# vliu15/3d-brain-tumor-segmentation

Hardware: AMD Instinct MI355X
Metric: training volumes/sec (2ch x 128^3) (higher is better)
Workload: dtype f32; 1 GPU; BASELINE configs[1]: 2ch x 128^3, batch 1 per GPU, fp32, full fwd+bwd with Dice+KL+L2 VAE loss + Dice metric + TF-form Adam; CLI-default model (base_filters=32, depth=4, groups=8, reduction=8; 42,174,773 params); parallelism=dp1, global_batch=1

## Files before the change

3d-brain-tumor-segmentation_amd/csrc/conv_igemm.hip:

```cpp
#include <stdlib.h>
#include "common.h"
#include "conv_plan.h"

#define MAXSLOT 8

int bts_prof_on();
void bts_prof_begin(int sym, double flops, hipStream_t stream);
void bts_prof_end(hipStream_t stream);

struct IgemmParams {
  const float* x;
  const float* wp;
  const float* bias;
  float* y;
  int N, Di, Hi, Wi, Cin, ldx;
  int Do, Ho, Wo;
  int Cout, ldy, Npad, KG;
  int ODa, OHa, OWa;
  int os, ooz, ooy, oox;
  int s, loz, loy, lox;
  int IZ, IY, IX;
  int lgTX, lgTY, TZ;
  int ntz, nty, ntx;
  int ntaps, flags;
// ... 811 lines not shown
#pragma unroll
    for (int i = 0; i < UPM_NSLOT; ++i) {
      f32x4 v = {0.f, 0.f, 0.f, 0.f};
      if (goff[i] >= 0) v = *reinterpret_cast<const f32x4*>(xbase + goff[i] + st * 8);
      pre[i] = v;
    }
  };
  auto commit = [&](float* buf) {
#pragma unroll
    for (int i = 0; i < UPM_NSLOT; ++i) {
      const int e = tid + i * 256;
      if (e < nslots) *reinterpret_cast<f32x4*>(buf + (e >> 1) * S + (e & 1) * 4) = pre[i];
    }
  };
  int kgBeg = 0, kgEnd = p.KG;
  if (p.ksplit > 1) {
    kgBeg = blockIdx.z * p.kg_per;
    kgEnd = kgBeg + p.kg_per;
    if (kgEnd > p.KG) kgEnd = p.KG;
  }
  fetch(kgBeg);
  commit(lds);
  __syncthreads();
  for (int st = kgBeg; st < kgEnd; ++st) {
    const float* cur = lds + ((st - kgBeg) & 1) * bufDw;
    const bool more = (st + 1) < kgEnd;
    if (more) fetch(st + 1);
    const float* wk = p.wp + st * wstepKG;
    constexpr int AD = 2;
    f32x4 a[AD + 1], bf[8];
#pragma unroll
    for (int q = 0; q < AD; ++q) a[q] = *reinterpret_cast<const f32x4*>((wk + q * wstepTap) + lane_woff);
#pragma unroll
    for (int o = 0; o < 8; ++o) bf[o] = *reinterpret_cast<const f32x4*>(cur + bbase + off8[o]);
#pragma unroll
    for (int t = 0; t < 27; ++t) {
      if (t + AD < 27) a[(t + AD) % (AD + 1)] = *reinterpret_cast<const f32x4*>((wk + (t + AD) * wstepTap) + lane_woff);
      __builtin_amdgcn_sched_barrier(0);
#pragma unroll
      for (int j = 0; j < 4; ++j)
        acc[upm_cls(t)] = __builtin_amdgcn_mfma_f32_32x32x2f32(a[t % (AD + 1)][j], bf[upm_off(t)][j], acc[upm_cls(t)], 0, 0, 0);
      __builtin_amdgcn_sched_barrier(0);
    }
    if (more) commit(lds + ((st + 1 - kgBeg) & 1) * bufDw);
    __syncthreads();
  }

  const int cz = cz0 + mz, cy = cy0 + my, cx = cx0 + mx;
  if (cz >= p.Di || cy >= p.Hi || cx >= p.Wi) return;
  const int nb = blockIdx.y * 32;
#pragma unroll
  for (int c = 0; c < 8; ++c) {
    const int oz = 2 * cz + ((c >> 2) & 1), oy = 2 * cy + ((c >> 1) & 1), ox = 2 * cx + (c & 1);
    const long vfine = (((long)n * (2 * p.Di) + oz) * (2 * p.Hi) + oy) * (2 * p.Wi) + ox;
    if (p.ksplit > 1) {
      float* row = p.part + ((long)blockIdx.z * ((long)p.N * 8 * p.Di * p.Hi * p.Wi) + vfine) * p.Npad;
#pragma unroll
      for (int g = 0; g < 4; ++g) {
        f32x4 v4 = {acc[c][4 * g + 0], acc[c][4 * g + 1], acc[c][4 * g + 2], acc[c][4 * g + 3]};
        *reinterpret_cast<f32x4*>(row + nb + 8 * g + 4 * h) = v4;
      }
      continue;
    }
    float* yrow = p.y + vfine * (long)p.ldy;
#pragma unroll
    for (int g = 0; g < 4; ++g) {
      const int co = nb + 8 * g + 4 * h;
      if (co >= p.Cout) continue;
      f32x4 v = {acc[c][4 * g + 0], acc[c][4 * g + 1], acc[c][4 * g + 2], acc[c][4 * g + 3]};
      if (p.flags & IG_FLAG_BIAS) {
#pragma unroll
        for (int j = 0; j < 4; ++j) v[j] += p.bias[co + j];
      }
      if (p.flags & IG_FLAG_SIGMOID) {
#pragma unroll
        for (int j = 0; j < 4; ++j) v[j] = sigmoidf_(v[j]);
      }
      f32x4* dst = reinterpret_cast<f32x4*>(yrow + co);
      if (p.flags & IG_FLAG_ACCUM) v += *dst;
      *dst = v;
    }
  }
}

static bool upm_accept(const ConvCall& c, ConvChoice& ch) {
  UpmPlan& u = ch.u;
  if ((c.ldx & 3) || (c.ldy & 3) || !c.x16 || !c.y16) return false;
  if ((c.Cin & 7) || (c.Cout & 3) || c.Wi < 8 || c.Hi < 4 || c.Di < 2) return false;
  const int Npad = npad32(c.Cout), KG = c.Cin / 8;
  int TX = 32;
  while (TX > 8 && TX / 2 >= c.Wi) TX /= 2;
  int TY = (TX == 32) ? 2 : 4;
  int TZ = 128 / (TX * TY);
  u.lgTX = ilog2(TX); u.lgTY = ilog2(TY); u.TZ = TZ;
  u.ntx = (c.Wi + TX - 1) / TX; u.nty = (c.Hi + TY - 1) / TY; u.ntz = (c.Di + TZ - 1) / TZ;
  u.IX = TX + 1; u.IY = TY + 1; u.IZ = TZ + 1;
  if (u.IZ * u.IY * u.IX * 2 > 256 * UPM_NSLOT) return false;
  const long wgs = (long)c.N * u.ntz * u.nty * u.ntx * (Npad / 32);
  const long min_wgs = conv_env_long("BTS_IGEMM_UPM_MIN", 256);
  u.ksplit = 1; u.kg_per = KG; u.need = 0;
  if (wgs < min_wgs) {
    if (KG < 8) return false;
    int ks = (int)((512 + wgs - 1) / wgs);
    if (ks > KG / 4) ks = KG / 4;
    if (ks > 16) ks = 16;
    if (ks < 2) return false;
    u.kg_per = (KG + ks - 1) / ks;
    u.ksplit = (KG + u.kg_per - 1) / u.kg_per;
    if (u.ksplit < 2 || wgs * u.ksplit < min_wgs / 2) return false;
    u.need = (long)u.ksplit * c.N * 8 * c.Di * c.Hi * c.Wi * Npad * 4;
  }
  ch.sym = 20;
  ch.ws = u.need;
  return c.ws_bytes >= u.need;
}

static int launch_upm(const ConvCall& c, const ConvChoice& ch, const ConvPtrs& q, hipStream_t stream) {
  const UpmPlan& u = ch.u;
  UpmParams p;
  p.N = c.N; p.Di = c.Di; p.Hi = c.Hi; p.Wi = c.Wi; p.Cin = c.Cin; p.Cout = c.Cout;
  p.Npad = npad32(c.Cout); p.KG = c.Cin / 8;
  p.lgTX = u.lgTX; p.lgTY = u.lgTY; p.TZ = u.TZ; p.ntx = u.ntx; p.nty = u.nty; p.ntz = u.ntz; p.IX = u.IX; p.IY = u.IY; p.IZ = u.IZ;
  p.ksplit = u.ksplit; p.kg_per = u.kg_per;
  p.x = q.x; p.wp = q.wp; p.bias = q.bias; p.y = q.y; p.ldx = c.ldx; p.ldy = c.ldy; p.flags = c.flags;
  p.part = reinterpret_cast<float*>(q.ws);
  const long tiles = (long)c.N * p.ntz * p.nty * p.ntx;
  const int ny = p.Npad / 32;
  const int tileVox = p.IZ * p.IY * p.IX;
  const size_t shmem = (size_t)2 * tileVox * 12 * sizeof(float);
  const bool prof = bts_prof_on();
  if (prof) bts_prof_begin(20, 2.0 * 27.0 * c.Cin * c.Cout * (double)c.N * c.Di * c.Hi * c.Wi, stream);
  (void)hipGetLastError(); hipLaunchKernelGGL(upm_kernel, dim3((unsigned)tiles, ny, p.ksplit), dim3(256), shmem, stream, p);
  if (prof) bts_prof_end(stream);
  BTS_LAUNCH_CHECK();
  if (p.ksplit > 1) {
    const long nvox = (long)c.N * 8 * c.Di * c.Hi * c.Wi;
    long blocks = (nvox * c.Cout + 255) / 256;
    if (blocks > 4096) blocks = 4096;
    (void)hipGetLastError(); hipLaunchKernelGGL(igemm_reduce_kernel, dim3((int)blocks), dim3(256), 0, stream, p.part, q.bias, q.y, nvox, c.Cout, p.Npad,
                       c.ldy, p.ksplit, p.flags);
    BTS_LAUNCH_CHECK();
  }
  return BTS_OK;
}

struct K1sParams {
  const float* x;
  const float* wp;
  const float* bias;
  float* y;
  long nvox;
  int Cin, ldx, Cout, ldy, Npad, KG, flags;
};
template <int NS>
__global__ __launch_bounds__(256, 4) void k1s_kernel(const K1sParams p) {
  const int lane = threadIdx.x & 63;
  const int wave = __builtin_amdgcn_readfirstlane(threadIdx.x >> 6);
  const int h = lane >> 5, l32 = lane & 31;
  const long v0 = (long)blockIdx.x * 256 + wave * 64;
  const float* xrow[2];
#pragma unroll
  for (int ms = 0; ms < 2; ++ms) {
    long v = v0 + ms * 32 + l32;
    if (v >= p.nvox) v = p.nvox - 1;
    xrow[ms] = p.x + v * p.ldx + h * 4;
  }
  int woff[NS];
#pragma unroll
  for (int ns = 0; ns < NS; ++ns) {
    int ncol = (blockIdx.y * NS + ns) * 32 + l32;
    if (ncol >= p.Npad) ncol = p.Npad - 1;
    woff[ns] = (h * p.Npad + ncol) * 4;
  }
  const int wstepKG = 2 * p.Npad * 4;
  f32x16 acc[2][NS];
#pragma unroll
  for (int ms = 0; ms < 2; ++ms)
#pragma unroll
    for (int ns = 0; ns < NS; ++ns)
#pragma unroll
      for (int r = 0; r < 16; ++r) acc[ms][ns][r] = 0.f;
  constexpr int U = (NS == 1) ? 2 : 1;
  f32x4 b[2][U][2], a[2][U][NS];
  auto load = [&](int buf, int kg) {
#pragma unroll
    for (int u = 0; u < U; ++u) {
      const int k = (kg + u < p.KG) ? kg + u : p.KG - 1;
#pragma unroll
      for (int ms = 0; ms < 2; ++ms) b[buf][u][ms] = *reinterpret_cast<const f32x4*>(xrow[ms] + k * 8);
#pragma unroll
      for (int ns = 0; ns < NS; ++ns) a[buf][u][ns] = *reinterpret_cast<const f32x4*>((p.wp + k * wstepKG) + woff[ns]);
    }
  };
  auto mma = [&](int buf, int kg) {
#pragma unroll
    for (int u = 0; u < U; ++u) {
      if (kg + u < p.KG) {
#pragma unroll
        for (int j = 0; j < 4; ++j)
#pragma unroll
          for (int ms = 0; ms < 2; ++ms)
#pragma unroll
            for (int ns = 0; ns < NS; ++ns)
              acc[ms][ns] = __builtin_amdgcn_mfma_f32_32x32x2f32(a[buf][u][ns][j], b[buf][u][ms][j], acc[ms][ns], 0, 0, 0);
      }
    }
  };
  load(0, 0);
  for (int kg = 0; kg < p.KG; kg += 2 * U) {
    if (kg + U < p.KG) load(1, kg + U);
    mma(0, kg);
    if (kg + U < p.KG) {
      if (kg + 2 * U < p.KG) load(0, kg + 2 * U);
      mma(1, kg + U);
    }
  }
#pragma unroll
  for (int ms = 0; ms < 2; ++ms) {
    const long v = v0 + ms * 32 + l32;
    if (v >= p.nvox) continue;
    float* yrow = p.y + v * p.ldy;
#pragma unroll
    for (int ns = 0; ns < NS; ++ns) {
      const int nb = (blockIdx.y * NS + ns) * 32;
#pragma unroll
      for (int g = 0; g < 4; ++g) {
        const int co = nb + 8 * g + 4 * h;
        if (co >= p.Cout) continue;
        f32x4 val = {acc[ms][ns][4 * g + 0], acc[ms][ns][4 * g + 1], acc[ms][ns][4 * g + 2], acc[ms][ns][4 * g + 3]};
        if (p.flags & IG_FLAG_BIAS) {
#pragma unroll
          for (int j = 0; j < 4; ++j)
            if (co + j < p.Cout) val[j] += p.bias[co + j];
        }
        if (p.flags & IG_FLAG_SIGMOID) {
#pragma unroll
          for (int j = 0; j < 4; ++j) val[j] = sigmoidf_(val[j]);
        }
        if ((p.flags & IG_FLAG_VECOUT) && co + 3 < p.Cout) {
          f32x4* dst = reinterpret_cast<f32x4*>(yrow + co);
          if (p.flags & IG_FLAG_ACCUM) val += *dst;
          *dst = val;
        } else {
#pragma unroll
          for (int j = 0; j < 4; ++j)
            if (co + j < p.Cout) yrow[co + j] = (p.flags & IG_FLAG_ACCUM) ? yrow[co + j] + val[j] : val[j];
        }
      }
    }
  }
}

static bool k1s_accept(const ConvCall& c, ConvChoice& ch) {
  if ((c.Cin & 7) || (c.ldx & 3) || !c.x16) return false;
  const long nvox = (long)c.N * c.Di * c.Hi * c.Wi;
  if (nvox < conv_env_long("BTS_IGEMM_K1S_MIN", 256 * 256)) return false;
  ch.sym = 21;
  return (nvox + 255) / 256 <= 0x7fffffffL;
}
static int launch_k1s(const ConvCall& c, const ConvChoice&, const ConvPtrs& q, hipStream_t stream) {
  K1sParams p;
  p.x = q.x; p.wp = q.wp; p.bias = q.bias; p.y = q.y; p.nvox = (long)c.N * c.Di * c.Hi * c.Wi;
  p.Cin = c.Cin; p.ldx = c.ldx; p.Cout = c.Cout; p.ldy = c.ldy; p.Npad = npad32(c.Cout); p.KG = c.Cin / 8;
  p.flags = c.flags;
  if ((c.ldy % 4 == 0) && c.y16) p.flags |= IG_FLAG_VECOUT;
  const long gx = (p.nvox + 255) / 256;
  const bool prof = bts_prof_on();
  const int ns = (p.Npad >= 64) ? 2 : 1;
  if (prof) bts_prof_begin(21, 2.0 * c.Cin * (double)c.Cout * (double)p.nvox, stream);
  (void)hipGetLastError();
  if (ns == 2) hipLaunchKernelGGL(k1s_kernel<2>, dim3((unsigned)gx, (p.Npad + 63) / 64), dim3(256), 0, stream, p);
  else hipLaunchKernelGGL(k1s_kernel<1>, dim3((unsigned)gx, 1), dim3(256), 0, stream, p);
  if (prof) bts_prof_end(stream);
  BTS_LAUNCH_CHECK();
  return BTS_OK;
}

struct DscParams {
  const float* x;
  const float* wp;
  const float* bias;
  float* y;
  int N, D, H, W, Cin, ldx, Cout, ldy, Npad, KG, ntx, nty, ntz, flags;
};
template <int CO>
__global__ __launch_bounds__(256, 4) void dsc_kernel(const DscParams p) {
  constexpr int S = 12, TX = 32, TY = 4, TZ = 2, IX = TX + 2, IY = TY + 2, IZ = TZ + 2;
  constexpr int tileVox = IZ * IY * IX, nslots = tileVox * 2, NSL = (nslots + 255) / 256;
  __shared__ __attribute__((aligned(16))) float lds[tileVox * S];
  const int tid = threadIdx.x;
  int b = blockIdx.x;
  const int tx = b % p.ntx; b /= p.ntx;
  const int ty = b % p.nty; b /= p.nty;
  const int tz = b % p.ntz;
  const int n = b / p.ntz;
  const int iz0 = tz * TZ - 1, iy0 = ty * TY - 1, ix0 = tx * TX - 1;
  const float* xbase = p.x + ((((long)n * p.D + iz0) * p.H + iy0) * p.W + ix0) * (long)p.ldx;
  int goff[NSL];
#pragma unroll
  for (int i = 0; i < NSL; ++i) {
    const int e = tid + i * 256;
    goff[i] = -1;
    if (e < nslots) {
      const int vox = e >> 1, q = e & 1;
      const int vz = vox / (IY * IX), r = vox - vz * (IY * IX), vy = r / IX, vx = r - vy * IX;
      if ((unsigned)(iz0 + vz) < (unsigned)p.D && (unsigned)(iy0 + vy) < (unsigned)p.H && (unsigned)(ix0 + vx) < (unsigned)p.W)
        goff[i] = ((vz * p.H + vy) * p.W + vx) * p.ldx + q * 4;
    }
  }
  const int mx = tid & (TX - 1), my = (tid >> 5) & (TY - 1), mz = tid >> 7;
  const float* lb = lds + ((mz * IY + my) * IX + mx) * S;
  float acc[CO];
#pragma unroll
  for (int c = 0; c < CO; ++c) acc[c] = 0.f;
  const int wstepKG = 2 * p.Npad * 4, wstepTap = p.KG * wstepKG;
  f32x4 pre[NSL];
  auto fetch = [&](int kg) {
#pragma unroll
    for (int i = 0; i < NSL; ++i) {
      f32x4 v = {0.f, 0.f, 0.f, 0.f};
      if (goff[i] >= 0) v = *reinterpret_cast<const f32x4*>(xbase + goff[i] + kg * 8);
      pre[i] = v;
    }
  };
  fetch(0);
  for (int kg = 0; kg < p.KG; ++kg) {
    __syncthreads();
#pragma unroll
    for (int i = 0; i < NSL; ++i) {
      const int e = tid + i * 256;
      if (e < nslots) *reinterpret_cast<f32x4*>(lds + (e >> 1) * S + (e & 1) * 4) = pre[i];
    }
    __syncthreads();
    if (kg + 1 < p.KG) fetch(kg + 1);
    const float* wk = p.wp + kg * wstepKG;
#pragma unroll
    for (int r = 0; r < 9; ++r) {
      float w[3][2][CO * 4];
#pragma unroll
      for (int dx = 0; dx < 3; ++dx)
#pragma unroll
        for (int hh = 0; hh < 2; ++hh)
#pragma unroll
          for (int q = 0; q < CO * 4; ++q) w[dx][hh][q] = wk[(r * 3 + dx) * wstepTap + hh * p.Npad * 4 + q];
      f32x4 xv[3][2];
#pragma unroll
      for (int dx = 0; dx < 3; ++dx) {
        const float* src = lb + (((r / 3) * IY + r % 3) * IX + dx) * S;
        xv[dx][0] = *reinterpret_cast<const f32x4*>(src);
        xv[dx][1] = *reinterpret_cast<const f32x4*>(src + 4);
      }
      __builtin_amdgcn_sched_barrier(0);
#pragma unroll
      for (int dx = 0; dx < 3; ++dx)
#pragma unroll
        for (int hh = 0; hh < 2; ++hh)
#pragma unroll
          for (int c = 0; c < CO; ++c)
#pragma unroll
            for (int j = 0; j < 4; ++j) acc[c] = fmaf(xv[dx][hh][j], w[dx][hh][c * 4 + j], acc[c]);
      __builtin_amdgcn_sched_barrier(0);
    }
  }
  const int oz = tz * TZ + mz, oy = ty * TY + my, ox = tx * TX + mx;
  if (oz >= p.D || oy >= p.H || ox >= p.W) return;
  float* yrow = p.y + ((((long)n * p.D + oz) * p.H + oy) * p.W + ox) * (long)p.ldy;
#pragma unroll
  for (int c = 0; c < CO; ++c) {
    if (c < p.Cout) {
      float v = acc[c];
      if (p.flags & IG_FLAG_BIAS) v += p.bias[c];
      if (p.flags & IG_FLAG_SIGMOID) v = sigmoidf_(v);
      if (p.flags & IG_FLAG_ACCUM) v += yrow[c];
      yrow[c] = v;
    }
  }
}

static bool dsc_accept(const ConvCall& c, ConvChoice& ch) {
  if (c.Cout > 4 || (c.Cin & 7) || (c.ldx & 3) || !c.x16) return false;
  const long tiles = (long)c.N * ((c.Di + 1) / 2) * ((c.Hi + 3) / 4) * ((c.Wi + 31) / 32);
  ch.sym = 22;
  return tiles >= conv_env_long("BTS_IGEMM_DSC_MIN", 1024) && tiles <= 0x7fffffffL;
}
static int launch_dsc(const ConvCall& c, const ConvChoice&, const ConvPtrs& q, hipStream_t stream) {
  DscParams p;
  p.x = q.x; p.wp = q.wp; p.bias = q.bias; p.y = q.y;
  p.N = c.N; p.D = c.Di; p.H = c.Hi; p.W = c.Wi; p.Cin = c.Cin; p.ldx = c.ldx; p.Cout = c.Cout; p.ldy = c.ldy;
  p.Npad = npad32(c.Cout); p.KG = c.Cin / 8;
  p.ntx = (c.Wi + 31) / 32; p.nty = (c.Hi + 3) / 4; p.ntz = (c.Di + 1) / 2;
  p.flags = c.flags;
  const long tiles = (long)c.N * p.ntz * p.nty * p.ntx;
  const bool prof = bts_prof_on();
  if (prof) bts_prof_begin(22, 2.0 * 27.0 * c.Cin * (double)c.Cout * (double)c.N * c.Di * c.Hi * c.Wi, stream);
  (void)hipGetLastError();
  if (c.Cout <= 2) hipLaunchKernelGGL(dsc_kernel<2>, dim3((unsigned)tiles), dim3(256), 0, stream, p);
  else hipLaunchKernelGGL(dsc_kernel<4>, dim3((unsigned)tiles), dim3(256), 0, stream, p);
  if (prof) bts_prof_end(stream);
  BTS_LAUNCH_CHECK();
  return BTS_OK;
}

struct C2Params {
  const float* x;
  const float* wp;
  const float* bias;
  float* y;
  const float* wp2;
  const float* bias2;
  float* y2;
  int N, D, H, W, ldx, Cout, ldy, ldy2, Npad;
  int ntz, nty, ntx;
  double* gnp;
  int gn_G, gn_zt;
};

template <bool F2>
__global__ __launch_bounds__(256, 2) void c2_kernel(const C2Params p) {
  __shared__ float lds[2 * 6 * 6 * 34 + 16];
  const int tid = threadIdx.x;
  const int lane = tid & 63;
  const int wave = __builtin_amdgcn_readfirstlane(tid >> 6);
  const int h = lane >> 5, l32 = lane & 31;
  int b = blockIdx.x;
  const int tx = b % p.ntx; b /= p.ntx;
// ... 592 lines not shown
```

3d-brain-tumor-segmentation_amd/csrc/conv_wgrad.hip:

```cpp
#include <stdlib.h>
#include <type_traits>
#include "common.h"
#include "bts_internal.h"

int bts_prof_on();
void bts_prof_begin(int sym, double flops, hipStream_t stream);
void bts_prof_end(hipStream_t stream);

#define WG_THREADS 512
#define WG_WAVES 8
#define WG_MAXT 4
#define WG_PSLOTS 8
#define WG_QSLOTS 4

struct WgradParams {
  const float* p;
  const float* q;
  float* partial;
  double* partial_b;
  const float* zeros;
  int N, Dp, Hp, Wp, Cp, ldp;
  int Dq, Hq, Wq, Cq, ldq;
  int s, loz, loy, lox;
  int IZ, IY, IX;
// ... 869 lines not shown
    for (int c = 0; c < 4; ++c)
#pragma unroll
      for (int r = 0; r < 16; ++r) acc[a][c][r] = 0.f;

  struct WgwOps {
    f32x4 v[4];
    f32x4 a0, a1, u1, u2;
    float a0s[2], a1s[2], u1s[2], u2s[2];
  };
  auto form = [&](const float* cur, auto stc, WgwOps& o) {
    constexpr int st = decltype(stc)::value;
    constexpr int py2 = st >> 1, sx = st & 1;
    const int xq = 2 * sx + hh;
    const int xo = 4 * xq;
    const int pq = (xq ^ pswz) << 2;
    f32x4 c[4];
#pragma unroll
    for (int yr = 0; yr < 4; ++yr) {
      const f32x4 a = *reinterpret_cast<const f32x4*>(cur + pA + (2 * py2 + yr) * 512 + pq);
      const f32x4 b = *reinterpret_cast<const f32x4*>(cur + pB + (2 * py2 + yr) * 512 + pq);
      c[yr] = wgw_fma4(b, sp2, a);
    }
    o.v[0] = wgw_sub4(c[0], c[2]);
    o.v[1] = wgw_add4(c[1], c[2]);
    o.v[2] = wgw_sub4(c[2], c[1]);
    o.v[3] = wgw_sub4(c[1], c[3]);
    const float* qb = cur + WGW_PTILE + ((2 * py2) * 32 + ch) * WGW_QSTR + xo;
    {
      const f32x4 x0q = *reinterpret_cast<const f32x4*>(qb + qX + 4);
      const f32x4 x1q = *reinterpret_cast<const f32x4*>(qb + qX + 32 * WGW_QSTR + 4);
      const f32x4 y0q = *reinterpret_cast<const f32x4*>(qb + (4 * 32) * WGW_QSTR + 4);
      const f32x4 y1q = *reinterpret_cast<const f32x4*>(qb + (5 * 32) * WGW_QSTR + 4);
      o.a0 = wgw_fma4(y0q, sq2, x0q);
      o.a1 = wgw_fma4(y1q, sq2, x1q);
      o.u1 = wgw_add4(o.a0, o.a1);
      o.u2 = wgw_sub4(o.a0, o.a1);
      if (bias) bsum += (double)((o.u1[0] + o.u1[1]) + (o.u1[2] + o.u1[3]));
    }
#pragma unroll
    for (int e = 0; e < 2; ++e) {
      const int off = e == 0 ? 0 : 8, el = e == 0 ? 3 : 0;
      f32x4 xs0 = *reinterpret_cast<const f32x4*>(qb + qX + off);
      f32x4 xs1 = *reinterpret_cast<const f32x4*>(qb + qX + 32 * WGW_QSTR + off);
      f32x4 ys0 = *reinterpret_cast<const f32x4*>(qb + (4 * 32) * WGW_QSTR + off);
      f32x4 ys1 = *reinterpret_cast<const f32x4*>(qb + (5 * 32) * WGW_QSTR + off);
      asm volatile("" : "+v"(xs0), "+v"(xs1), "+v"(ys0), "+v"(ys1));
      o.a0s[e] = fmaf(ys0[el], sq, xs0[el]);
      o.a1s[e] = fmaf(ys1[el], sq, xs1[el]);
      o.u1s[e] = o.a0s[e] + o.a1s[e];
      o.u2s[e] = o.a0s[e] - o.a1s[e];
    }
  };
  auto mfma48 = [&](const WgwOps& o) {
#pragma unroll
    for (int dx = 0; dx < 3; ++dx)
#pragma unroll
      for (int j = 0; j < 4; ++j) {
        const int w = 5 + j - dx;
        const float b0 = w == 3 ? o.a0s[0] : w == 8 ? o.a0s[1] : o.a0[(w - 4) & 3];
        const float b1 = w == 3 ? o.u1s[0] : w == 8 ? o.u1s[1] : o.u1[(w - 4) & 3];
        const float b2 = w == 3 ? o.u2s[0] : w == 8 ? o.u2s[1] : o.u2[(w - 4) & 3];
        const float b3 = w == 3 ? o.a1s[0] : w == 8 ? o.a1s[1] : o.a1[(w - 4) & 3];
        acc[dx][0] = __builtin_amdgcn_mfma_f32_32x32x2f32(o.v[0][j], b0, acc[dx][0], 0, 0, 0);
        acc[dx][1] = __builtin_amdgcn_mfma_f32_32x32x2f32(o.v[1][j], b1, acc[dx][1], 0, 0, 0);
        acc[dx][2] = __builtin_amdgcn_mfma_f32_32x32x2f32(o.v[2][j], b2, acc[dx][2], 0, 0, 0);
        acc[dx][3] = __builtin_amdgcn_mfma_f32_32x32x2f32(o.v[3][j], b3, acc[dx][3], 0, 0, 0);
      }
  };
#define WGW_SCHED_STEP()                                   \
  _Pragma("unroll") for (int q_ = 0; q_ < 48; ++q_) {      \
    __builtin_amdgcn_sched_group_barrier(0x008, 1, 0);     \
    __builtin_amdgcn_sched_group_barrier(0x002, 2, 0);     \
    __builtin_amdgcn_sched_group_barrier(0x320, 1, 0);     \
  }

  const int t0 = blockIdx.x * p.sub_per_wg;
  int t1 = t0 + p.sub_per_wg;
  if (t1 > p.nsub) t1 = p.nsub;
  if (t0 < t1) {
    fetch_begin();
    fetch_quarter(IC<0>{}); fetch_quarter(IC<1>{}); fetch_quarter(IC<2>{}); fetch_quarter(IC<3>{});
    commit_quarter(lds, IC<0>{}); commit_quarter(lds, IC<1>{}); commit_quarter(lds, IC<2>{}); commit_quarter(lds, IC<3>{});
  }
  __syncthreads();
  WgwOps opA, opB;
  for (int t = t0; t < t1; ++t) {
    const float* cur = lds + ((t - t0) & 1) * WGW_BUF;
    float* nxt = lds + ((t - t0 + 1) & 1) * WGW_BUF;
    const bool more = (t + 1) < t1;
    form(cur, IC<0>{}, opA);
    if (more) fetch_begin();
    __builtin_amdgcn_sched_barrier(0);
    asm volatile("s_nop 3" ::: "memory");
    if (more) fetch_quarter(IC<0>{});
    form(cur, IC<1>{}, opB);
    mfma48(opA);
    WGW_SCHED_STEP();
    __builtin_amdgcn_sched_barrier(0);
    asm volatile("s_nop 1" ::: "memory");
    if (more) { commit_quarter(nxt, IC<0>{}); fetch_quarter(IC<1>{}); }
    form(cur, IC<2>{}, opA);
    mfma48(opB);
    WGW_SCHED_STEP();
    __builtin_amdgcn_sched_barrier(0);
    asm volatile("s_nop 1" ::: "memory");
    if (more) { commit_quarter(nxt, IC<1>{}); fetch_quarter(IC<2>{}); }
    form(cur, IC<3>{}, opB);
    mfma48(opA);
    WGW_SCHED_STEP();
    __builtin_amdgcn_sched_barrier(0);
    asm volatile("s_nop 1" ::: "memory");
    if (more) { commit_quarter(nxt, IC<2>{}); fetch_quarter(IC<3>{}); }
    mfma48(opB);
    WGW_SCHED_STEP();
    __builtin_amdgcn_sched_barrier(0);
    if (more) commit_quarter(nxt, IC<3>{});
    __syncthreads();
  }

  asm volatile("s_nop 15\n\ts_nop 15\n\ts_nop 15\n\ts_nop 15\n\ts_nop 15" ::: "memory");
  float* xl = lds + wave * 9 * 1024;
#pragma unroll
  for (int dx = 0; dx < 3; ++dx)
#pragma unroll
    for (int r = 0; r < 16; ++r) {
      const float u0 = wgw_acc_rd(acc[dx][0][r]), u1 = wgw_acc_rd(acc[dx][1][r]), u2 = wgw_acc_rd(acc[dx][2][r]),
                  u3 = wgw_acc_rd(acc[dx][3][r]);
      const float hs = 0.5f * (u1 + u2), hd = 0.5f * (u1 - u2);
      const int crow = 8 * (r >> 2) + 4 * hh + (r & 3);
      float* o = xl + (dx * 3) * 1024 + crow * 32 + ch;
      o[0] = u0 + hs;
      o[1024] = hd;
      o[2048] = hs - u3;
    }
  __syncthreads();
  float* out = p.partial + ((((long)blockIdx.x * gridDim.y + pct) * gridDim.z + qct) * 27) * 1024;
  for (int e = tid; e < 9 * 1024; e += WGW_THREADS) {
    const int g = e >> 10, ck = e & 1023;
    const int dx = g / 3, ky = g - dx * 3;
    const float l0 = lds[(0 * 9 + g) * 1024 + ck], l1 = lds[(1 * 9 + g) * 1024 + ck], l2 = lds[(2 * 9 + g) * 1024 + ck],
                l3 = lds[(3 * 9 + g) * 1024 + ck];
    const float hs = 0.5f * (l1 + l2), hd = 0.5f * (l1 - l2);
    out[((0 * 3 + ky) * 3 + dx) * 1024 + ck] = l0 + hs;
    out[((1 * 3 + ky) * 3 + dx) * 1024 + ck] = hd;
    out[((2 * 3 + ky) * 3 + dx) * 1024 + ck] = hs - l3;
  }
  if (bias) {
    const double o = __shfl_xor(bsum, 32, 64);
    if (lane < 32) p.partial_b[((long)blockIdx.x * gridDim.z + qct) * 32 + ch] = bsum + o;
  }
}

#define K1W_THREADS 512
#define K1W_U 8
__global__ __launch_bounds__(K1W_THREADS, 2) void k1w_kernel(const WgradParams p, long NV, long chunk) {
  __shared__ float lds[8 * 1024];
  const int tid = threadIdx.x;
  const int lane = tid & 63;
  const int wave = __builtin_amdgcn_readfirstlane(tid >> 6);
  const int ch = lane & 31, hh = lane >> 5;
  const int pct = blockIdx.y, qct = blockIdx.z;
  const int pc = pct * 32 + ch, qc = qct * 32 + ch;
  const bool pok = pc < p.Cp, qok = qc < p.Cq;
  const long w0 = (long)blockIdx.x * chunk;
  long w1 = w0 + chunk;
  if (w1 > NV) w1 = NV;
  long per = ((w1 - w0 + 7) / 8 + 1) & ~1L;
  long v = w0 + wave * per;
  long ve = v + per;
  if (ve > w1) ve = w1;
  f32x16 acc;
#pragma unroll
  for (int r = 0; r < 16; ++r) acc[r] = 0.f;
  double bsum = 0.0;
  const bool bias = p.want_bias && pct == 0;
  const float* pp = p.p + pc;
  const float* qq = p.q + qc;
  for (; v < ve; v += 2 * K1W_U) {
    float a[K1W_U], b[K1W_U];
#pragma unroll
    for (int u = 0; u < K1W_U; ++u) {
      const long vv = v + 2 * u + hh;
      const bool in = vv < ve;
      a[u] = (in && pok) ? pp[vv * p.ldp] : 0.f;
      b[u] = (in && qok) ? qq[vv * p.ldq] : 0.f;
    }
    float bs = 0.f;
#pragma unroll
    for (int u = 0; u < K1W_U; ++u) {
      acc = __builtin_amdgcn_mfma_f32_32x32x2f32(a[u], b[u], acc, 0, 0, 0);
      bs += b[u];
    }
    if (bias) bsum += (double)bs;
  }
#pragma unroll
  for (int r = 0; r < 16; ++r) lds[wave * 1024 + ((r & 3) + 8 * (r >> 2) + 4 * hh) * 32 + ch] = acc[r];
  __syncthreads();
  float* dst = p.partial + ((((long)blockIdx.x * gridDim.y + pct) * gridDim.z + qct) * p.ntiles) * 1024;
  for (int e = tid; e < 1024; e += K1W_THREADS) {
    float sacc = lds[e];
#pragma unroll
    for (int w = 1; w < 8; ++w) sacc += lds[w * 1024 + e];
    dst[e] = sacc;
  }
  if (bias) {
    __syncthreads();
    double* shd = reinterpret_cast<double*>(lds);
    shd[tid] = bsum;
    __syncthreads();
    if (tid < 32) {
      double t = 0.0;
      for (int k = 0; k < 16; ++k) t += shd[k * 32 + tid];
      p.partial_b[((long)blockIdx.x * gridDim.z + qct) * 32 + tid] = t;
    }
  }
}

struct WgradRoles {
  int ntaps, s, neg, swapped, transposed;
  int Dp, Hp, Wp, Cp, Dq, Hq, Wq, Cq;
};

static int wgrad_roles(WgradRoles& r, int kind, int D, int H, int W, int Cin, int Cout) {
  r.ntaps = (kind == BTS_CONV_K1) ? 1 : 27;
  r.s = 1; r.neg = 0; r.swapped = 0; r.transposed = 0;
  r.Dp = D; r.Hp = H; r.Wp = W; r.Cp = Cin; r.Dq = D; r.Hq = H; r.Wq = W; r.Cq = Cout;
  if (kind == BTS_CONV_K3S2) {
    if ((D | H | W) & 1) return BTS_ERR_SHAPE;
    r.s = 2; r.Dq = D / 2; r.Hq = H / 2; r.Wq = W / 2;
  } else if (kind == BTS_CONV_K3S2T) {
    r.transposed = 1;
    r.s = 2; r.Dp = 2 * D; r.Hp = 2 * H; r.Wp = 2 * W; r.Cp = Cout; r.Cq = Cin;
  } else if (kind == BTS_CONV_K3S1 && Cout <= 8 && Cin > Cout) {
    r.swapped = 1; r.neg = 1; r.Cp = Cout; r.Cq = Cin;
  }
  return BTS_OK;
}

extern "C" int bts_colsum(const float* x, float* out, void* workspace, long workspace_bytes, int N, long rows, int C,
                          int ld, float scale, int sum_over_n, int accumulate, hipStream_t stream);
extern "C" long bts_colsum_workspace(int N, long rows, int C);

extern "C" long bts_conv3d_bwd_weight_workspace(int kind, int N, int D, int H, int W, int Cin, int Cout) {
  WgradRoles r;
  if (wgrad_roles(r, kind, D, H, W, Cin, Cout) != BTS_OK) return -1;
  WgradPlan pl;
  if (plan_wgrad(pl, r.ntaps, r.s, r.neg, N, r.Dp, r.Hp, r.Wp, r.Cp, r.Dq, r.Hq, r.Wq, r.Cq) != BTS_OK) return -1;
  const long base = ((pl.partial_floats * 4 + pl.partial_b_doubles * 8 + 256 + 15) & ~15L);
  return base + (r.swapped ? bts_colsum_workspace(N, (long)D * H * W, Cout) : 0) + 128;
}

extern "C" int bts_conv3d_bwd_weight(int kind, const float* x, const float* dy, float* dw, float* db, void* workspace,
                                     long workspace_bytes, int N, int D, int H, int W, int Cin, int ldx, int Cout,
                                     int lddy, int dup_start, int dup_shift, int accumulate, hipStream_t stream) {
  WgradRoles ro;
  int r = wgrad_roles(ro, kind, D, H, W, Cin, Cout);
  if (r != BTS_OK) return r;
  if (dup_shift > 0 && (kind == BTS_CONV_K3S2 || kind == BTS_CONV_K3S2T)) return BTS_ERR_UNSUPPORTED;
  WgradPlan pl;
  r = plan_wgrad(pl, ro.ntaps, ro.s, ro.neg, N, ro.Dp, ro.Hp, ro.Wp, ro.Cp, ro.Dq, ro.Hq, ro.Wq, ro.Cq);
  if (r != BTS_OK) return r;
  const long need = bts_conv3d_bwd_weight_workspace(kind, N, D, H, W, Cin, Cout);
  if (workspace_bytes < need || workspace == nullptr) return BTS_ERR_WORKSPACE;
  WgradParams& p = pl.p;
  const bool pIsDy = ro.transposed || ro.swapped;
  p.p = pIsDy ? dy : x;
  p.q = pIsDy ? x : dy;
  p.ldp = pIsDy ? lddy : ldx;
  p.ldq = pIsDy ? ldx : lddy;
  p.partial = reinterpret_cast<float*>(workspace);
  uintptr_t pb = (uintptr_t)(p.partial + pl.partial_floats);
  pb = (pb + 15) & ~(uintptr_t)15;
  p.partial_b = reinterpret_cast<double*>(pb);
  p.want_bias = (db != nullptr && !pIsDy) ? 1 : 0;
  typedef void (*WgKernel)(const WgradParams);
  static const WgKernel kernels[4] = {wgrad_kernel<0, 0>, wgrad_kernel<1, 0>, wgrad_kernel<2, 1>, wgrad_kernel<2, 2>};
  static bool attr_done = false;
  if (!attr_done) {
    for (int i = 0; i < 4; ++i) {
      hipError_t e = hipFuncSetAttribute(reinterpret_cast<const void*>(kernels[i]), hipFuncAttributeMaxDynamicSharedMemorySize, 160 * 1024);
      if (e != hipSuccess) return (int)e;
    }
    attr_done = true;
  }
  char* ztail = reinterpret_cast<char*>(workspace) + ((need - 64) & ~15L);
  p.zeros = reinterpret_cast<const float*>(ztail);
  const bool glds = (p.ldp % 4 == 0) && (p.Cp % 4 == 0) && ((((uintptr_t)p.p) & 15) == 0) && (p.ldq % 4 == 0) &&
                    (p.Cq % 4 == 0) && ((((uintptr_t)p.q) & 15) == 0);
  if (p.fastf && ((double)p.IZ * p.Hp * p.Wp * p.ldp * 4.0 >= 4.0e9 || (double)p.TZ * p.Hq * p.Wq * p.ldq * 4.0 >= 4.0e9 || !glds))
    p.fastf = p.fixg = 0;
  const bool prof = bts_prof_on();
  if (glds && !p.fastf) {
    hipError_t e = hipMemsetAsync(ztail, 0, 64, stream);
    if (e != hipSuccess) return (int)e;
  }
  const int kidx = !glds ? 0 : (p.fastf ? 1 + p.fixg : 1);
  bool use_wgw = false;
  if (kidx == 2 && ro.ntaps == 27 && ro.s == 1) {
    const char* e = getenv("BTS_WGW");
    use_wgw = !(e && atoi(e) == 0) && 5.0 * p.Hp * p.Wp * p.ldp * 4.0 < 2.0e9 && 3.0 * p.Hq * p.Wq * p.ldq * 4.0 < 2.0e9;
  }
  bool use_k1w = false;
  const long NVall = (long)N * ro.Dq * ro.Hq * ro.Wq;
  if (ro.ntaps == 1 && !pIsDy && p.ntiles == 1 && NVall >= 32768) {
    const char* e = getenv("BTS_K1W");
    use_k1w = !(e && atoi(e) == 0);
  }
  if (use_k1w) {
    const long chunk = (((NVall + pl.nsp - 1) / pl.nsp) + 15) & ~15L;
    if (prof) bts_prof_begin(26, 2.0 * (double)ro.Cp * ro.Cq * (double)NVall, stream);
    (void)hipGetLastError();
    hipLaunchKernelGGL(k1w_kernel, dim3(pl.nsp, pl.npct, pl.nqct), dim3(K1W_THREADS), 0, stream, p, NVall, chunk);
    if (prof) bts_prof_end(stream);
    BTS_LAUNCH_CHECK();
  } else if (use_wgw) {
    static bool wattr = false;
    if (!wattr) {
      hipError_t e = hipFuncSetAttribute(reinterpret_cast<const void*>(wgw_kernel), hipFuncAttributeMaxDynamicSharedMemorySize, 160 * 1024);
      if (e != hipSuccess) return (int)e;
      wattr = true;
    }
    if (prof) bts_prof_begin(24, 2.0 * ro.ntaps * (double)ro.Cp * ro.Cq * (double)N * ro.Dq * ro.Hq * ro.Wq, stream);
    (void)hipGetLastError();
    hipLaunchKernelGGL(wgw_kernel, dim3(pl.nsp, pl.npct, pl.nqct), dim3(WGW_THREADS), (size_t)2 * WGW_BUF * sizeof(float), stream, p);
    if (prof) bts_prof_end(stream);
    BTS_LAUNCH_CHECK();
  } else {
  static const int ksym[4] = {100, 104, 109, 110};
  if (prof) bts_prof_begin(ksym[kidx], 2.0 * ro.ntaps * (double)ro.Cp * ro.Cq * (double)N * ro.Dq * ro.Hq * ro.Wq, stream);
  (void)hipGetLastError(); hipLaunchKernelGGL(kernels[kidx], dim3(pl.nsp, pl.npct, pl.nqct), dim3(WG_THREADS), pl.shmem, stream, p);
  if (prof) bts_prof_end(stream);
  BTS_LAUNCH_CHECK();
  }
  WfinParams f;
  f.partial = p.partial; f.partial_b = p.partial_b; f.dw = dw; f.db = p.want_bias ? db : nullptr;
  f.nsp = pl.nsp; f.npct = pl.npct; f.nqct = pl.nqct; f.ntaps = ro.ntaps; f.ntiles = p.ntiles; f.cpad = p.cpad;
  f.Cp = ro.Cp; f.Cq = ro.Cq;
  const int Cin_ref = Cin + dup_shift;
  f.sT = (long)Cin_ref * Cout;
  if (ro.transposed) { f.sP = Cin_ref; f.sQ = 1; f.fold_axis = 0; }
  else if (ro.swapped) { f.sP = 1; f.sQ = Cout; f.fold_axis = 2; }
  else { f.sP = Cout; f.sQ = 1; f.fold_axis = 1; }
  f.shift = dup_shift;
  f.dup_start = dup_shift > 0 ? dup_start : (1 << 30);
  f.accum = accumulate;
  long rows = (long)ro.ntaps * ro.Cp * pl.nqct;
  if (pl.nsp <= 16) {
    long blocks = (rows * 32 + 255) / 256;
    if (blocks > 8192) blocks = 8192;
    (void)hipGetLastError(); hipLaunchKernelGGL(wgrad_finalize_flat_kernel, dim3((int)blocks), dim3(256), 0, stream, f);
  } else {
    int blocks = (int)(rows < 4096 ? rows : 4096);
    (void)hipGetLastError(); hipLaunchKernelGGL(wgrad_finalize_kernel, dim3(blocks), dim3(256), 0, stream, f);
  }
  BTS_LAUNCH_CHECK();
  if (db != nullptr && ro.swapped) {
    char* cw = reinterpret_cast<char*>(workspace) + ((pl.partial_floats * 4 + pl.partial_b_doubles * 8 + 256 + 15) & ~15L);
    const long rowsv = (long)D * H * W;
    return bts_colsum(dy, db, cw, bts_colsum_workspace(N, rowsv, Cout), N, rowsv, Cout, lddy, 1.0f, 1, accumulate, stream);
  }
  return BTS_OK;
}
```

Before: 27.29 volumes/s.

## Restructure 1x1 conv kernels: hold B in registers, pipeline A loads, XCD-aware wgrad mapping

```diff
diff --git a/3d-brain-tumor-segmentation_amd/csrc/conv_igemm.hip b/3d-brain-tumor-segmentation_amd/csrc/conv_igemm.hip
--- a/3d-brain-tumor-segmentation_amd/csrc/conv_igemm.hip
+++ b/3d-brain-tumor-segmentation_amd/csrc/conv_igemm.hip
@@ -987,82 +987,66 @@
   long nvox;
   int Cin, ldx, Cout, ldy, Npad, KG, flags;
 };
-template <int NS>
+template <int NS, int KH>
 __global__ __launch_bounds__(256, 4) void k1s_kernel(const K1sParams p) {
+  constexpr bool HOLD = (NS == 1);
+  constexpr int RA = HOLD ? (KH == 8 ? 2 : 4) : KH;
+  constexpr int OB = HOLD ? (KH == 8 ? 2 : 4) : 2;
   const int lane = threadIdx.x & 63;
   const int wave = __builtin_amdgcn_readfirstlane(threadIdx.x >> 6);
   const int h = lane >> 5, l32 = lane & 31;
   const long v0 = (long)blockIdx.x * 256 + wave * 64;
   const float* xrow[2];
+  float* ycur[2];
+  bool vok[2];
 #pragma unroll
   for (int ms = 0; ms < 2; ++ms) {
     long v = v0 + ms * 32 + l32;
-    if (v >= p.nvox) v = p.nvox - 1;
+    vok[ms] = v < p.nvox;
+    if (!vok[ms]) v = p.nvox - 1;
     xrow[ms] = p.x + v * p.ldx + h * 4;
-  }
-  int woff[NS];
-#pragma unroll
-  for (int ns = 0; ns < NS; ++ns) {
-    int ncol = (blockIdx.y * NS + ns) * 32 + l32;
-    if (ncol >= p.Npad) ncol = p.Npad - 1;
-    woff[ns] = (h * p.Npad + ncol) * 4;
-  }
+    ycur[ms] = p.y + v * p.ldy + h * 4 + blockIdx.y * (32 * NS);
+  }
+  int co0 = blockIdx.y * (32 * NS) + h * 4;
   const int wstepKG = 2 * p.Npad * 4;
-  f32x16 acc[2][NS];
-#pragma unroll
-  for (int ms = 0; ms < 2; ++ms)
-#pragma unroll
-    for (int ns = 0; ns < NS; ++ns)
-#pragma unroll
-      for (int r = 0; r < 16; ++r) acc[ms][ns][r] = 0.f;
-  constexpr int U = (NS == 1) ? 2 : 1;
-  f32x4 b[2][U][2], a[2][U][NS];
-  auto load = [&](int buf, int kg) {
-#pragma unroll
-    for (int u = 0; u < U; ++u) {
-      const int k = (kg + u < p.KG) ? kg + u : p.KG - 1;
-#pragma unroll
-      for (int ms = 0; ms < 2; ++ms) b[buf][u][ms] = *reinterpret_cast<const f32x4*>(xrow[ms] + k * 8);
-#pragma unroll
-      for (int ns = 0; ns < NS; ++ns) a[buf][u][ns] = *reinterpret_cast<const f32x4*>((p.wp + k * wstepKG) + woff[ns]);
-    }
+  const unsigned aoff = (h * p.Npad + l32) * 4;
+  const int lastcb = p.Npad / 32 - 1;
+  f32x4 b[KH][2], a[RA][NS];
+  auto loadB = [&](int slot, int k) {
+#pragma unroll
+    for (int ms = 0; ms < 2; ++ms) b[slot][ms] = *reinterpret_cast<const f32x4*>(xrow[ms] + k * 8);
   };
-  auto mma = [&](int buf, int kg) {
-#pragma unroll
-    for (int u = 0; u < U; ++u) {
-      if (kg + u < p.KG) {
-#pragma unroll
-        for (int j = 0; j < 4; ++j)
-#pragma unroll
-          for (int ms = 0; ms < 2; ++ms)
-#pragma unroll
-            for (int ns = 0; ns < NS; ++ns)
-              acc[ms][ns] = __builtin_amdgcn_mfma_f32_32x32x2f32(a[buf][u][ns][j], b[buf][u][ms][j], acc[ms][ns], 0, 0, 0);
-      }
+  auto loadA = [&](int slot, int cb, int k) {
+#pragma unroll
+    for (int ns = 0; ns < NS; ++ns) {
+      const int c32 = (cb * NS + ns < lastcb) ? cb * NS + ns : lastcb;
+      const float* wk = p.wp + (long)k * wstepKG + c32 * 128;
+      a[slot][ns] = *reinterpret_cast<const f32x4*>(wk + aoff);
     }
   };
-  load(0, 0);
-  for (int kg = 0; kg < p.KG; kg += 2 * U) {
-    if (kg + U < p.KG) load(1, kg + U);
-    mma(0, kg);
-    if (kg + U < p.KG) {
-      if (kg + 2 * U < p.KG) load(0, kg + 2 * U);
-      mma(1, kg + U);
-    }
-  }
-#pragma unroll
-  for (int ms = 0; ms < 2; ++ms) {
-    const long v = v0 + ms * 32 + l32;
-    if (v >= p.nvox) continue;
-    float* yrow = p.y + v * p.ldy;
-#pragma unroll
-    for (int ns = 0; ns < NS; ++ns) {
-      const int nb = (blockIdx.y * NS + ns) * 32;
-#pragma unroll
-      for (int g = 0; g < 4; ++g) {
-        const int co = nb + 8 * g + 4 * h;
-        if (co >= p.Cout) continue;
-        f32x4 val = {acc[ms][ns][4 * g + 0], acc[ms][ns][4 * g + 1], acc[ms][ns][4 * g + 2], acc[ms][ns][4 * g + 3]};
+  const bool vec = (p.flags & IG_FLAG_VECOUT) != 0, accum = (p.flags & IG_FLAG_ACCUM) != 0;
+  const bool rdold = vec && accum && p.Cout >= 4;
+  auto store_tile = [&](const f32x16& c, int ms, int d0) {
+#pragma unroll
+    for (int q0 = 0; q0 < 4; q0 += OB) {
+      __builtin_amdgcn_sched_barrier(0);
+      f32x4 old[OB];
+#pragma unroll
+      for (int i = 0; i < OB; ++i) old[i] = f32x4{0.f, 0.f, 0.f, 0.f};
+      if (rdold) {
+#pragma unroll
+        for (int i = 0; i < OB; ++i) {
+          const int d = d0 + 8 * (q0 + i);
+          old[i] = *reinterpret_cast<const f32x4*>(ycur[ms] + ((co0 + d + 3 < p.Cout) ? d : -co0));
+        }
+      }
+#pragma unroll
+      for (int i = 0; i < OB; ++i) {
+        const int g = q0 + i, d = d0 + 8 * g;
+        const int co = co0 + d;
+        if (!vok[ms] || co >= p.Cout) continue;
+        float* yq = ycur[ms] + d;
+        f32x4 val = {c[4 * g + 0], c[4 * g + 1], c[4 * g + 2], c[4 * g + 3]};
         if (p.flags & IG_FLAG_BIAS) {
 #pragma unroll
           for (int j = 0; j < 4; ++j)
@@ -1072,17 +1056,86 @@
 #pragma unroll
           for (int j = 0; j < 4; ++j) val[j] = sigmoidf_(val[j]);
         }
-        if ((p.flags & IG_FLAG_VECOUT) && co + 3 < p.Cout) {
-          f32x4* dst = reinterpret_cast<f32x4*>(yrow + co);
-          if (p.flags & IG_FLAG_ACCUM) val += *dst;
-          *dst = val;
+        if (vec && co + 3 < p.Cout) {
+          if (accum) val += old[i];
+          *reinterpret_cast<f32x4*>(yq) = val;
         } else {
 #pragma unroll
           for (int j = 0; j < 4; ++j)
-            if (co + j < p.Cout) yrow[co + j] = (p.flags & IG_FLAG_ACCUM) ? yrow[co + j] + val[j] : val[j];
+            if (co + j < p.Cout) yq[j] = accum ? yq[j] + val[j] : val[j];
         }
       }
     }
+  };
+#pragma unroll
+  for (int s = 0; s < RA; ++s) {
+    loadA(s, blockIdx.y, s < p.KG ? s : p.KG - 1);
+    __builtin_amdgcn_sched_barrier(0);
+  }
+#pragma unroll
+  for (int s = 0; s < KH; ++s) {
+    loadB(s, s < p.KG ? s : p.KG - 1);
+    __builtin_amdgcn_sched_barrier(0);
+  }
+  if constexpr (HOLD) {
+    const int nblk = p.Npad / 32;
+    for (int blk = 0; blk < nblk; ++blk) {
+#pragma unroll
+      for (int ms = 0; ms < 2; ++ms) {
+        f32x16 acc;
+#pragma unroll
+        for (int r = 0; r < 16; ++r) acc[r] = 0.f;
+#pragma unroll
+        for (int s = 0; s < KH; ++s) {
+          if (s < p.KG) {
+#pragma unroll
+            for (int j = 0; j < 4; ++j) acc = __builtin_amdgcn_mfma_f32_32x32x2f32(a[s % RA][0][j], b[s][ms][j], acc, 0, 0, 0);
+            if (s + RA < p.KG) loadA(s % RA, blk, s + RA);
+          }
+        }
+        __builtin_amdgcn_sched_barrier(0);
+        if (ms == 0 || blk + 1 < nblk) {
+#pragma unroll
+          for (int s = 0; s < RA; ++s) loadA(s, blk + ms, s < p.KG ? s : p.KG - 1);
+        }
+        store_tile(acc, ms, 0);
+        __builtin_amdgcn_sched_barrier(0);
+      }
+#pragma unroll
+      for (int ms = 0; ms < 2; ++ms) ycur[ms] += 32;
+      co0 += 32;
+    }
+  } else {
+    const int cb = blockIdx.y;
+    f32x16 acc[2][NS];
+#pragma unroll
+    for (int ms = 0; ms < 2; ++ms)
+#pragma unroll
+      for (int ns = 0; ns < NS; ++ns)
+#pragma unroll
+        for (int r = 0; r < 16; ++r) acc[ms][ns][r] = 0.f;
+    for (int kg0 = 0; kg0 < p.KG; kg0 += KH) {
+#pragma unroll
+      for (int s = 0; s < KH; ++s) {
+        const int kg = kg0 + s;
+        if (kg < p.KG) {
+#pragma unroll
+          for (int j = 0; j < 4; ++j)
+#pragma unroll
+            for (int ms = 0; ms < 2; ++ms)
+#pragma unroll
+              for (int ns = 0; ns < NS; ++ns)
+                acc[ms][ns] = __builtin_amdgcn_mfma_f32_32x32x2f32(a[s % RA][ns][j], b[s][ms][j], acc[ms][ns], 0, 0, 0);
+          if (kg + RA < p.KG) loadA(s % RA, cb, kg + RA);
+          if (kg + KH < p.KG) loadB(s, kg + KH);
+        }
+      }
+    }
+    __builtin_amdgcn_sched_barrier(0);
+#pragma unroll
+    for (int ms = 0; ms < 2; ++ms)
+#pragma unroll
+      for (int ns = 0; ns < NS; ++ns) store_tile(acc[ms][ns], ms, ns * 32);
   }
 }
 
@@ -1101,11 +1154,11 @@
   if ((c.ldy % 4 == 0) && c.y16) p.flags |= IG_FLAG_VECOUT;
   const long gx = (p.nvox + 255) / 256;
   const bool prof = bts_prof_on();
-  const int ns = (p.Npad >= 64) ? 2 : 1;
   if (prof) bts_prof_begin(21, 2.0 * c.Cin * (double)c.Cout * (double)p.nvox, stream);
   (void)hipGetLastError();
-  if (ns == 2) hipLaunchKernelGGL(k1s_kernel<2>, dim3((unsigned)gx, (p.Npad + 63) / 64), dim3(256), 0, stream, p);
-  else hipLaunchKernelGGL(k1s_kernel<1>, dim3((unsigned)gx, 1), dim3(256), 0, stream, p);
+  if (p.KG <= 4) hipLaunchKernelGGL((k1s_kernel<1, 4>), dim3((unsigned)gx, 1), dim3(256), 0, stream, p);
+  else if (p.KG <= 8) hipLaunchKernelGGL((k1s_kernel<1, 8>), dim3((unsigned)gx, 1), dim3(256), 0, stream, p);
+  else hipLaunchKernelGGL((k1s_kernel<2, 3>), dim3((unsigned)gx, (p.Npad + 63) / 64), dim3(256), 0, stream, p);
   if (prof) bts_prof_end(stream);
   BTS_LAUNCH_CHECK();
   return BTS_OK;
diff --git a/3d-brain-tumor-segmentation_amd/csrc/conv_wgrad.hip b/3d-brain-tumor-segmentation_amd/csrc/conv_wgrad.hip
--- a/3d-brain-tumor-segmentation_amd/csrc/conv_wgrad.hip
+++ b/3d-brain-tumor-segmentation_amd/csrc/conv_wgrad.hip
@@ -1045,17 +1045,22 @@
 }
 
 #define K1W_THREADS 512
-#define K1W_U 8
-__global__ __launch_bounds__(K1W_THREADS, 2) void k1w_kernel(const WgradParams p, long NV, long chunk) {
+#define K1W_U 32
+__global__ __launch_bounds__(K1W_THREADS, 2) void k1w_kernel(const WgradParams p, long NV, long chunk, int nsp, int npct, int nqct) {
   __shared__ float lds[8 * 1024];
   const int tid = threadIdx.x;
   const int lane = tid & 63;
   const int wave = __builtin_amdgcn_readfirstlane(tid >> 6);
   const int ch = lane & 31, hh = lane >> 5;
-  const int pct = blockIdx.y, qct = blockIdx.z;
+  const int pairs = npct * nqct;
+  const int xcd = blockIdx.x & 7, slot = blockIdx.x >> 3;
+  const int total = nsp * pairs;
+  const int item = xcd * (total >> 3) + (xcd < (total & 7) ? xcd : (total & 7)) + slot;
+  const int sp = item / pairs;
+  const int pct = (item % pairs) / nqct, qct = (item % pairs) % nqct;
   const int pc = pct * 32 + ch, qc = qct * 32 + ch;
   const bool pok = pc < p.Cp, qok = qc < p.Cq;
-  const long w0 = (long)blockIdx.x * chunk;
+  const long w0 = (long)sp * chunk;
   long w1 = w0 + chunk;
   if (w1 > NV) w1 = NV;
   long per = ((w1 - w0 + 7) / 8 + 1) & ~1L;
@@ -1078,18 +1083,21 @@
       a[u] = (in && pok) ? pp[vv * p.ldp] : 0.f;
       b[u] = (in && qok) ? qq[vv * p.ldq] : 0.f;
     }
-    float bs = 0.f;
-#pragma unroll
-    for (int u = 0; u < K1W_U; ++u) {
-      acc = __builtin_amdgcn_mfma_f32_32x32x2f32(a[u], b[u], acc, 0, 0, 0);
-      bs += b[u];
-    }
-    if (bias) bsum += (double)bs;
+#pragma unroll
+    for (int u0 = 0; u0 < K1W_U; u0 += 8) {
+      float bs = 0.f;
+#pragma unroll
+      for (int u = u0; u < u0 + 8; ++u) {
+        acc = __builtin_amdgcn_mfma_f32_32x32x2f32(a[u], b[u], acc, 0, 0, 0);
+        bs += b[u];
+      }
+      if (bias) bsum += (double)bs;
+    }
   }
 #pragma unroll
   for (int r = 0; r < 16; ++r) lds[wave * 1024 + ((r & 3) + 8 * (r >> 2) + 4 * hh) * 32 + ch] = acc[r];
   __syncthreads();
-  float* dst = p.partial + ((((long)blockIdx.x * gridDim.y + pct) * gridDim.z + qct) * p.ntiles) * 1024;
+  float* dst = p.partial + ((((long)sp * npct + pct) * nqct + qct) * p.ntiles) * 1024;
   for (int e = tid; e < 1024; e += K1W_THREADS) {
     float sacc = lds[e];
 #pragma unroll
@@ -1104,7 +1112,7 @@
     if (tid < 32) {
       double t = 0.0;
       for (int k = 0; k < 16; ++k) t += shd[k * 32 + tid];
-      p.partial_b[((long)blockIdx.x * gridDim.z + qct) * 32 + tid] = t;
+      p.partial_b[((long)sp * nqct + qct) * 32 + tid] = t;
     }
   }
 }
@@ -1203,7 +1211,8 @@
     const long chunk = (((NVall + pl.nsp - 1) / pl.nsp) + 15) & ~15L;
     if (prof) bts_prof_begin(26, 2.0 * (double)ro.Cp * ro.Cq * (double)NVall, stream);
     (void)hipGetLastError();
-    hipLaunchKernelGGL(k1w_kernel, dim3(pl.nsp, pl.npct, pl.nqct), dim3(K1W_THREADS), 0, stream, p, NVall, chunk);
+    const long wgs = (long)pl.nsp * pl.npct * pl.nqct;
+    hipLaunchKernelGGL(k1w_kernel, dim3((unsigned)wgs), dim3(K1W_THREADS), 0, stream, p, NVall, chunk, pl.nsp, pl.npct, pl.nqct);
     if (prof) bts_prof_end(stream);
     BTS_LAUNCH_CHECK();
   } else if (use_wgw) {
```

Result: no change. 27.33 volumes/s, median of 6 (+0.2%).
